# bobzhangbo2012/gnss-sdr-new

Measured on AMD Instinct MI355X. Metric: IQ Msamples/s processed (acq+track), 32 PRN × 81 Doppler; % HBM roofline, higher is better.
Workload: dtype f32; 1 GPU; C2: GPS L1 C/A 4 Msps; per 1 ms block a 32 PRN x 81 Doppler (+-10 kHz, 250 Hz) CFAR PCPS grid + closed-loop DLL/PLL tracking (3-tap E-P-L, dll_pll_veml_tracking) of 8 channels over the same span; fs_sps=4000000, fft_size=4000, prns=32, doppler_bins=81, channels=8, taps=3, item_type=gr_complex, tracking=one continuous stream, one launch per timed region, acq_chains=2, acq_stagger=0, acq_input=each step acquires its own span of the continuous stream (new HBM addresses), carrier=exact, forward_spectra_per_block=4

## Files before the change

gnss-sdr-new_amd/csrc/acq.hip:

```cpp
#include <algorithm>
#include <cmath>
#include <cstring>
#include <memory>
#include <new>
#include <utility>

#include "acq_handle.h"
#include "acq_plans.h"
#include "gsdr_stream_internal.h"

using namespace gsdr_acq_impl;

namespace
{

int dispatch(gsdr_acq* a, const AcqView& v, const AcqOp& op)
{
    if (a->variant >= 20) return dispatch_four(a, v, op);
    if (a->variant >= 10) return dispatch_runtime(a, v, op);
    return dispatch_static(a, v, op);
}

int run_blocks(gsdr_acq* a, const AcqView& v, const void* iq, uint32_t nblocks, uint64_t stride, uint64_t stamp0,
    gsdr_acq_result* res, hipStream_t s)
// ... 4 lines not shown
int run_ring(gsdr_acq* a, gsdr_stream* ring, uint64_t first_sample, uint32_t nblocks, uint64_t stamp0)
{
    gsdr::StreamReader rd(ring);
    const void* iq = nullptr;
    int rc = rd.view(first_sample, (uint64_t)nblocks * a->K * a->consumed, &iq);
    if (rc == GSDR_OK) rc = rd.acquire(a->stream);
    if (rc == GSDR_OK) rc = run_blocks(a, view_of(a), iq, nblocks, a->consumed, stamp0, a->d_res, a->stream);
    if (rc == GSDR_OK) rc = rd.release(a->stream);
    return rc;
}

int read_results(gsdr_acq* a, gsdr_acq_result* out, size_t n)
{
    GSDR_HIP(hipMemcpyAsync(out, a->d_res, n * sizeof(gsdr_acq_result), hipMemcpyDeviceToHost, a->stream));
    GSDR_HIP(hipStreamSynchronize(a->stream));
    return GSDR_OK;
}

int code_fft(gsdr_acq* a, uint32_t first_slot, uint32_t nslots)
{
    AcqOp op{AcqOp::CodeFft};
    op.first_slot = first_slot;
    op.nslots = nslots;
    return dispatch(a, view_of(a), op);
}

void step_two_freqs(const gsdr_acq* a, float center, float* freqs)
{
    const uint32_t nb = a->st2.nbins;
    const float half = (float)std::floor((double)nb / 2.0);
    for (uint32_t d = 0; d < nb; ++d)
        {
            volatile float dop = ((float)d - half) * a->st2.step;
            freqs[d] = center + dop;
        }
}

hipError_t upload_twiddles(float2* d_tw, uint32_t n)
{
    std::vector<float2> tw(n);
    for (uint32_t m = 0; m < n; ++m)
        {
            const double ang = 2.0 * M_PI * (double)m / (double)n;
            tw[m] = make_float2((float)std::cos(ang), (float)(-std::sin(ang)));
        }
    return hipMemcpy(d_tw, tw.data(), (size_t)n * sizeof(float2), hipMemcpyHostToDevice);
}
// ... 102 lines not shown
            a->eff = N / 2;
        }
    a->general = a->K > 1 || conf->bit_transition_flag;
    a->D = conf->num_doppler_bins;
    if (a->D == 0)
        a->D = (uint32_t)std::ceil((double)(conf->doppler_max - (-conf->doppler_max)) / (double)conf->doppler_step);
    GSDR_REQUIRE(a->D != 0, GSDR_E_ARG, "gsdr_acq_create: zero Doppler bins");
    const bool ok = choose_variant(a);
    const bool four = a->variant >= 20;
    a->lds_bytes = (size_t)(four ? a->plan4.sub.n : N) * sizeof(float2) + 16 * sizeof(RowStat);
    GSDR_REQUIRE(ok && a->lds_bytes <= kLdsBytes, GSDR_E_UNSUPPORTED,
        "gsdr_acq_create: FFT size %u not supported (needs 2^a*3^b*5^c; up to 20352 points in LDS, larger sizes as "
        "R*N2 with R in {8,10,12,16,20,25} and N2 <= 20352)", N);
    int rc = dispatch(a, view_of(a), AcqOp{AcqOp::SetAttrs});
    if (rc == GSDR_OK && four) rc = setup_split(a);
    if (rc == GSDR_OK && !a->general && default_pk_variant(N) > 0)
        rc = setup_corr_variant(a, a->env.corr_variant >= 0 ? a->env.corr_variant : default_pk_variant(N));
    if (rc != GSDR_OK) return rc;
    const size_t nP = conf->max_prns, nB = conf->max_blocks;
    hipError_t e = hipStreamCreateWithFlags(&a->stream, hipStreamNonBlocking);
    if (e == hipSuccess) e = hipMalloc(&a->d_tw, (size_t)N * sizeof(float2));
    if (e == hipSuccess) e = hipMalloc(&a->d_wipe, (size_t)a->D * N * sizeof(float2));
    if (e == hipSuccess) e = hipMalloc(&a->d_code_fft, nP * N * sizeof(float2));
    if (e == hipSuccess) e = hipMalloc(&a->d_code_stage, nP * a->consumed * sizeof(float2));
    if (e == hipSuccess) e = hipMalloc(&a->d_prn, nP * sizeof(uint32_t));
    if (e == hipSuccess) e = hipMalloc(&a->d_X, nB * a->K * a->D * N * sizeof(float2));
    if (e == hipSuccess) e = hipMalloc(&a->d_stats, nB * nP * a->K * a->D * sizeof(RowStat));
    if (e == hipSuccess) e = hipMalloc(&a->d_res, nB * nP * sizeof(gsdr_acq_result));
    if (e == hipSuccess) e = hipMalloc(&a->d_iq, nB * a->K * a->consumed * gsdr::item_bytes(conf->item_type));
    if (a->general)
        {
            const int nslots = 256 * 32 / (a->nt / 64);
            a->acc_words = (nslots + 31) / 32;
            if (e == hipSuccess) e = hipMalloc(&a->d_resk, nB * nP * a->K * sizeof(gsdr_acq_result));
            if (e == hipSuccess) e = hipMalloc(&a->d_acc, (size_t)a->acc_words * 32 * a->eff * sizeof(float));
            if (e == hipSuccess) e = hipMalloc(&a->d_acc_slots, (size_t)a->acc_words * sizeof(uint32_t));
            if (e == hipSuccess) e = hipMemset(a->d_acc_slots, 0, (size_t)a->acc_words * sizeof(uint32_t));
        }
    if (e == hipSuccess) e = hipMalloc(&a->d_grid, (size_t)a->D * N * sizeof(float));
    if (e == hipSuccess && a->split > 0 && !(conf->pfa > 0.0f))
        e = hipMalloc(&a->d_rowbuf, nB * nP * N * sizeof(float));
    if (e == hipSuccess && a->split > 0) e = hipMalloc(&a->d_keys, nB * nP * sizeof(unsigned long long));
    if (e == hipSuccess && a->split > 0) e = hipMalloc(&a->d_psum, nB * nP * 4 * sizeof(float));
    if (e == hipSuccess && a->split > 0) e = hipMalloc(&a->d_fscratch, nB * a->K * a->D * N * sizeof(float2));
    if (four)
        {
// ... 16 lines not shown
    rc = rebuild_wipeoffs(a);
    if (rc != GSDR_OK) return rc;
    compute_threshold(a);
    *out = guard.release();
    return GSDR_OK;
}

void gsdr_acq_destroy(gsdr_acq* a)
{
    if (!a) return;
    gsdr::DeviceGuard g(a->device);
    if (a->stream) (void)hipStreamSynchronize(a->stream);
    for (auto& r : a->prof_recs)
        {
            (void)hipEventDestroy(r.a);
            (void)hipEventDestroy(r.b);
        }
    for (hipEvent_t e : a->prof_pool) (void)hipEventDestroy(e);
    for (int i = 0; i < gsdr_acq::kSubs; ++i)
        {
            if (a->sub_done[i]) (void)hipEventDestroy(a->sub_done[i]);
            if (a->h_res[i]) (void)hipHostFree(a->h_res[i]);
        }
    void* bufs[] = {a->st2.d_wipe, a->st2.d_freq, a->d_tw, a->d_wipe, a->d_code_fft, a->d_code_stage, a->d_prn, a->d_X, a->d_stats, a->d_res,
        a->d_iq, a->d_grid, a->d_rowbuf, a->d_keys, a->d_psum, a->d_fscratch, a->d_dgrid, a->d_tw_sub, a->d_scratch, a->d_slots, a->d_resk, a->d_acc, a->d_acc_slots};
    for (void* p : bufs)
        if (p) (void)hipFree(p);
    if (a->stream) (void)hipStreamDestroy(a->stream);
    delete a;
}

int gsdr_acq_get_dims(const gsdr_acq* a, uint32_t* D, uint32_t* N)
{
    GSDR_REQUIRE(a, GSDR_E_ARG, "gsdr_acq_get_dims: null handle");
    if (D) *D = a->D;
    if (N) *N = a->N;
    return GSDR_OK;
}

int gsdr_acq_get_plan(const gsdr_acq* a, int32_t* variant, int32_t* nthreads, int32_t* r1, int32_t* nstages,
    int32_t radix[8])
{
    GSDR_REQUIRE(a, GSDR_E_ARG, "gsdr_acq_get_plan: null handle");
    static_assert(gsdr::fft::kMaxStages == 8, "gsdr_acq_get_plan reports 8 radices");
    const bool four = a->variant >= 20;
    const Plan& p = four ? a->plan4.sub : a->plan;
    if (variant) *variant = a->variant;
// ... 265 lines not shown
    float* grid_host)
{
    GSDR_REQUIRE(a && iq_host && grid_host, GSDR_E_ARG, "gsdr_acq_dump_grid_step_two: null argument");
    GSDR_REQUIRE(prn_slot < a->nprn, GSDR_E_ARG, "gsdr_acq_dump_grid_step_two: prn_slot %u >= nprn %u", prn_slot,
        a->nprn);
    GSDR_REQUIRE(a->st2.nbins > 0, GSDR_E_STATE, "gsdr_acq_dump_grid_step_two: gsdr_acq_set_step_two first");
    GSDR_REQUIRE(a->st2.nbins <= a->D, GSDR_E_UNSUPPORTED,
        "gsdr_acq_dump_grid_step_two: %u narrow bins exceed the grid buffer's %u rows", a->st2.nbins, a->D);
    std::lock_guard<std::mutex> lk(a->mu);
    gsdr::DeviceGuard g(a->device);
    const uint32_t nb = a->st2.nbins;
    std::vector<float> freqs(nb);
    step_two_freqs(a, doppler_center_hz, freqs.data());
    GSDR_HIP(hipMemcpyAsync(a->d_iq, iq_host, (size_t)a->consumed * gsdr::item_bytes(a->conf.item_type),
        hipMemcpyHostToDevice, a->stream));
    GSDR_HIP(hipMemcpyAsync(a->st2.d_freq, freqs.data(), nb * sizeof(float), hipMemcpyHostToDevice, a->stream));
    int rc = launch_wipeoff(a, a->st2.d_wipe, nb, a->st2.d_freq);
    if (rc != GSDR_OK) return rc;
    AcqView v = view_of(a);
    v.D = nb;
    v.nprn = 1;
    v.wipe = a->st2.d_wipe;
    v.code_fft = a->d_code_fft + (size_t)prn_slot * a->N;
    v.xm = XMap{nb, 0u, a->N};
    rc = dispatch(a, v, AcqOp{AcqOp::DumpGrid});
    if (rc != GSDR_OK) return rc;
    GSDR_HIP(hipMemcpyAsync(grid_host, a->d_grid, (size_t)nb * a->N * sizeof(float), hipMemcpyDeviceToHost,
        a->stream));
    GSDR_HIP(hipStreamSynchronize(a->stream));
    return GSDR_OK;
}

int gsdr_acq_set_step_two(gsdr_acq* a, uint32_t num_doppler_bins_step2, float doppler_step2, float pfa2)
{
    GSDR_REQUIRE(a, GSDR_E_ARG, "gsdr_acq_set_step_two: null handle");
    GSDR_REQUIRE(num_doppler_bins_step2 > 0, GSDR_E_ARG, "gsdr_acq_set_step_two: zero bins");
    GSDR_REQUIRE(num_doppler_bins_step2 <= a->D * a->conf.max_blocks, GSDR_E_UNSUPPORTED,
        "gsdr_acq_set_step_two: %u bins exceed the handle's spectrum capacity (%u bins x %u blocks)",
        num_doppler_bins_step2, a->D, a->conf.max_blocks);
    std::lock_guard<std::mutex> lk(a->mu);
    gsdr::DeviceGuard g(a->device);
    GSDR_HIP(hipStreamSynchronize(a->stream));
    if (a->st2.d_wipe) (void)hipFree(a->st2.d_wipe);
    if (a->st2.d_freq) (void)hipFree(a->st2.d_freq);
    a->st2.d_wipe = nullptr;
    a->st2.d_freq = nullptr;
// ... 19 lines not shown
{
    GSDR_REQUIRE(a && iq_host && prn_slots && doppler_center_hz && coarse_input_power && out, GSDR_E_ARG,
        "gsdr_acq_run_step_two: null argument");
    GSDR_REQUIRE(a->st2.nbins > 0, GSDR_E_STATE, "gsdr_acq_run_step_two: gsdr_acq_set_step_two first");
    GSDR_REQUIRE(nsel > 0 && nsel <= a->nprn, GSDR_E_ARG, "gsdr_acq_run_step_two: %u PRNs outside [1,%u]", nsel,
        a->nprn);
    for (uint32_t i = 0; i < nsel; ++i)
        GSDR_REQUIRE(prn_slots[i] < a->nprn, GSDR_E_ARG, "gsdr_acq_run_step_two: slot %u >= nprn %u", prn_slots[i],
            a->nprn);
    std::lock_guard<std::mutex> lk(a->mu);
    gsdr::DeviceGuard g(a->device);
    const uint32_t nb = a->st2.nbins;
    std::vector<float> freqs((size_t)nsel * nb);
    for (uint32_t i = 0; i < nsel; ++i) step_two_freqs(a, doppler_center_hz[i], freqs.data() + (size_t)i * nb);
    GSDR_HIP(hipMemcpyAsync(a->d_iq, iq_host, (size_t)a->K * a->consumed * gsdr::item_bytes(a->conf.item_type),
        hipMemcpyHostToDevice, a->stream));
    GSDR_HIP(hipMemcpyAsync(a->st2.d_freq, freqs.data(), freqs.size() * sizeof(float), hipMemcpyHostToDevice,
        a->stream));
    int rc = launch_wipeoff(a, a->st2.d_wipe, nsel * nb, a->st2.d_freq);
    const float thr = step_two_threshold(a);
    for (uint32_t i = 0; i < nsel && rc == GSDR_OK; ++i)
        {
            const AcqView v{nb, 1, a->st2.d_wipe + (size_t)i * nb * a->N, a->d_code_fft + (size_t)prn_slots[i] * a->N,
                a->d_prn + prn_slots[i], XMap{nb, 0u, a->N}, true, doppler_center_hz[i], coarse_input_power[i], thr};
            rc = run_blocks(a, v, a->d_iq, 1, a->consumed, stamp, a->d_res + i, a->stream);
        }
    if (rc != GSDR_OK) return rc;
    return read_results(a, out, nsel);
}

int gsdr_acq_set_cu_mask(gsdr_acq* a, const uint32_t* mask, int n_words)
{
    GSDR_REQUIRE(a, GSDR_E_ARG, "gsdr_acq_set_cu_mask: null handle");
    std::lock_guard<std::mutex> lk(a->mu);
    gsdr::DeviceGuard g(a->device);
    return gsdr::replace_stream(&a->stream, mask, n_words);
}

int gsdr_acq_set_profiling(gsdr_acq* a, int enable)
{
    GSDR_REQUIRE(a, GSDR_E_ARG, "gsdr_acq_set_profiling: null handle");
    std::lock_guard<std::mutex> lk(a->mu);
    a->profiling = enable != 0;
    if (a->profiling)
        {
            gsdr::DeviceGuard g(a->device);
            while (a->prof_pool.size() + 2 * a->prof_recs.size() < 1024)
// ... 96 lines not shown
```

gnss-sdr-new_amd/csrc/acq_common.hip:

```cpp
#include <cmath>
#include <cstdlib>
#include <string>

#include "acq_handle.h"

namespace
{

__device__ __forceinline__ float2 cephes_sincos_avx2(float x0)
{
    const float FOPI = 1.27323954473516f;
    const float DP1 = -0.78515625f, DP2 = -2.4187564849853515625e-4f, DP3 = -3.77489497744594108e-8f;
    const float C0 = 2.443315711809948E-005f, C1 = -1.388731625493765E-003f, C2 = 4.166664568298827E-002f;
    const float S0 = -1.9515295891E-4f, S1 = 8.3321608736E-3f, S2 = -1.6666654611E-1f;
    const uint32_t bits = __float_as_uint(x0);
    bool sign_sin = (bits >> 31) != 0;
    float x = __uint_as_float(bits & 0x7fffffffu);
    float y = __fmul_rn(x, FOPI);
    int32_t j = (int32_t)y;
    j = (j + 1) & ~1;
    y = (float)j;
    const bool swap = (j & 4) != 0;
    const bool poly = (j & 2) == 0;
    x = __fadd_rn(x, __fmul_rn(y, DP1));
// ... 152 lines not shown
                    const float acc = s[opp].sum;
                    const float ip = ap.step_two ? ap.ip2
                                                 : (float)((double)(acc / (float)(int32_t)ap.eff) / 2.0 / (double)(k + 1));
                    r.input_power = ip;
                    r.test_statistic = m / ip;
                    r.positive = r.test_statistic > ap.threshold ? 1 : 0;
                    done = r.positive || k + 1 == K;
                    if (done && threadIdx.x == 0) res[bp] = r;
                }
            if (threadIdx.x == 0) resk[(size_t)bp * K + k] = r;
        }
}

__global__ void acq_decide_kernel(const gsdr_acq_result* __restrict__ resk, gsdr_acq_result* __restrict__ res,
    uint32_t K, uint32_t n)
{
    const uint32_t bp = blockIdx.x * blockDim.x + threadIdx.x;
    if (bp >= n) return;
    uint32_t k = 0;
    while (k + 1 < K && !resk[(size_t)bp * K + k].positive) ++k;
    res[bp] = resk[(size_t)bp * K + k];
}

__global__ void __launch_bounds__(256) acq_grid_second_peak_kernel(const float* __restrict__ grid,
    gsdr_acq_result* __restrict__ res, AcqParams ap)
{
    __shared__ RowStat scratch[4];
    const uint32_t p = blockIdx.x;
    const uint32_t d = res[p].doppler_index;
    const int32_t ti = (int32_t)res[p].code_phase;
    const int32_t E = (int32_t)ap.N;
    int32_t e1 = ti - (int32_t)ap.samples_per_chip;
    int32_t e2 = ti + (int32_t)ap.samples_per_chip;
    if (e1 < 0)
        e1 = E + e1;
    else if (e2 >= E)
        e2 = e2 - E;
    const float* row = grid + ((size_t)p * ap.D + d) * ap.eff;
    float best = 0.0f, sum = 0.0f;
    uint32_t bidx = 0;
    for (uint32_t j = threadIdx.x; j < ap.eff; j += 256)
        {
            const int32_t jj = (int32_t)j;
            const bool excluded = (e1 < e2) ? (jj >= e1 && jj < e2) : (jj >= e1 || jj < e2);
            const float m = excluded ? 0.0f : row[j];
            if (stat_better(m, j, best, bidx))
// ... 90 lines not shown
#define GSDR_ACQ_QPW_DEFAULT 2
#endif

AcqEnv read_acq_env()
{
    AcqEnv e;
    if (const char* w = std::getenv("GSDR_ACQ_WIPE"))
        {
            const std::string m(w);
            e.wipe_mode = m == "generic" ? GSDR_WIPE_GENERIC : (m == "avx2" ? GSDR_WIPE_AVX2 : GSDR_WIPE_EXACT);
        }
    e.xshift = env_int("GSDR_ACQ_XSHIFT", 1) != 0;
    e.four_generic = env_int("GSDR_ACQ_FOUR_GENERIC", 0) != 0;
    e.split = env_int("GSDR_ACQ_SPLIT", 1) != 0;
    e.split_arg = env_int("GSDR_ACQ_SPLIT_ARG", 1) != 0;
    e.qpw = env_int("GSDR_ACQ_QPW", GSDR_ACQ_QPW_DEFAULT);
    e.ppw = env_int("GSDR_ACQ_PPW", GSDR_ACQ_PPW_DEFAULT);
    e.corr_variant = env_int("GSDR_ACQ_CORR_VARIANT", -1);
    return e;
}

AcqView view_of(const gsdr_acq* a)
{
    return AcqView{a->D, a->nprn, a->d_wipe, a->d_code_fft, a->d_prn, a->xm, false, 0.0f, 0.0f, 0.0f};
}

AcqParams params_of(const gsdr_acq* a, const AcqView& v)
{
    AcqParams ap{};
    ap.xm = v.xm;
    ap.N = a->N;
    ap.consumed = a->consumed;
    ap.lead_zeros = a->lead;
    ap.D = v.D;
    ap.P = v.nprn;
    ap.doppler_max = a->conf.doppler_max;
    ap.doppler_center = a->conf.doppler_center;
    ap.doppler_step = (int32_t)a->conf.doppler_step;
    ap.samples_per_code = a->conf.samples_per_code;
    ap.samples_per_chip = a->conf.samples_per_chip;
    ap.dwells = a->K;
    ap.threshold = a->threshold;
    ap.cfar = a->conf.pfa > 0.0f ? 1 : 0;
    ap.eff = a->eff;
    ap.out_off = a->N - a->eff;
    ap.counter = a->K;
    if (v.step_two)
// ... 51 lines not shown
    return GSDR_OK;
}

int launch_reduce(gsdr_acq* a, const AcqParams& ap, bool dwells, uint32_t nblocks, gsdr_acq_result* res,
    const uint32_t* prn, uint64_t stamp0, uint64_t stride, hipStream_t s)
{
    if (dwells)
        hipLaunchKernelGGL(acq_reduce_dwell_kernel, dim3(nblocks * ap.P), dim3(64), 0, s, a->d_stats, a->d_resk, res,
            prn, ap, stamp0, stride);
    else
        hipLaunchKernelGGL(acq_reduce_kernel, dim3(nblocks * ap.P), dim3(64), 0, s, a->d_stats, res, prn, ap, stamp0,
            stride);
    GSDR_HIP(hipGetLastError());
    return GSDR_OK;
}

int launch_decide(gsdr_acq* a, uint32_t n, gsdr_acq_result* res, hipStream_t s)
{
    hipLaunchKernelGGL(acq_decide_kernel, dim3((n + 255) / 256), dim3(256), 0, s, a->d_resk, res, a->K, n);
    GSDR_HIP(hipGetLastError());
    return GSDR_OK;
}

int launch_grid_second_peak(gsdr_acq* a, const AcqParams& ap, gsdr_acq_result* res, hipStream_t s)
{
    hipLaunchKernelGGL(acq_grid_second_peak_kernel, dim3(ap.P), dim3(256), 0, s, a->d_dgrid, res, ap);
    GSDR_HIP(hipGetLastError());
    return GSDR_OK;
}

void compute_threshold(gsdr_acq* a)
{
    const float pfa = a->conf.pfa;
    if (pfa <= 0.0f) return;
    const int num_bins = (int)(a->eff * a->D);
    const double p = std::pow(1.0 - (double)pfa, 1.0 / (double)(float)num_bins);
    a->threshold = (float)(2.0 * gsdr::gamma_p_inv_int(2 * (int)a->conf.max_dwells, p));
}

float step_two_threshold(const gsdr_acq* a)
{
    const float pfa = a->st2.pfa2;
    if (pfa <= 0.0f) return a->threshold;
    const int num_bins = (int)(a->eff * a->st2.nbins);
    const double p = std::pow(1.0 - (double)pfa, 1.0 / (double)(float)num_bins);
    return (float)(2.0 * gsdr::gamma_p_inv_int(2 * (int)a->conf.max_dwells, p));
// ... 4 lines not shown
```

gnss-sdr-new_amd/csrc/acq_handle.h:

```cpp
#pragma once
#include <mutex>
#include <type_traits>
#include <vector>

#include "acq_kernels.h"

struct AcqEnv
{
    int wipe_mode{GSDR_WIPE_EXACT};
    bool xshift{true}, four_generic{false}, split{true}, split_arg{true};
    int qpw{0}, ppw{0};
    int corr_variant{-1};
};

struct gsdr_acq
{
    int device{0};
    gsdr_acq_conf conf{};
    AcqEnv env{};
    uint32_t N{0}, D{0}, consumed{0}, lead{0};
    uint32_t K{1};
    int wipe_mode{GSDR_WIPE_EXACT};
    gsdr_acq_impl::XMap xm{};
    uint32_t eff{0};
    bool general{false};
    gsdr_acq_result* d_resk{nullptr};
    float* d_acc{nullptr};
    uint32_t* d_acc_slots{nullptr};
    int acc_words{0};
    float threshold{0.0f};
    int nt{256};
    int variant{0};
    int corr_variant{0};
    int split{0};
    int corr_stat{0};
    size_t corr_lds_bytes{0};
    gsdr::fft::Plan plan{};
    gsdr::fft::Plan4 plan4{};
    size_t lds_bytes{0};
    hipStream_t stream{nullptr};
    float2* d_tw{nullptr};
    float2* d_wipe{nullptr};
    float2* d_code_fft{nullptr};
    float2* d_code_stage{nullptr};
    uint32_t* d_prn{nullptr};
    uint32_t nprn{0};
    float2* d_X{nullptr};
    gsdr_acq_impl::RowStat* d_stats{nullptr};
    gsdr_acq_result* d_res{nullptr};
    static constexpr int kSubs = 2;
    gsdr_acq_result* h_res[kSubs]{};
    hipEvent_t sub_done[kSubs]{};
    uint32_t sub_blocks[kSubs]{}, sub_nprn[kSubs]{};
    int sub_head{0}, sub_count{0};
    void* d_iq{nullptr};
    float* d_grid{nullptr};
    float* d_rowbuf{nullptr};
    unsigned long long* d_keys{nullptr};
    float* d_psum{nullptr};
    float2* d_fscratch{nullptr};
    float* d_dgrid{nullptr};
    float2* d_tw_sub{nullptr};
    float2* d_scratch{nullptr};
    uint32_t* d_slots{nullptr};
    struct ProfRec
    {
// ... 2 lines not shown
    };
    bool profiling{false};
    std::vector<ProfRec> prof_recs;
    std::vector<hipEvent_t> prof_pool;
    struct StepTwo
    {
        uint32_t nbins{0};
        float step{0.0f};
        float pfa2{0.0f};
        float2* d_wipe{nullptr};
        float* d_freq{nullptr};
    } st2;
    std::mutex mu;
};

namespace gsdr_acq_impl
{

struct AcqView
{
    uint32_t D, nprn;
    const float2* wipe;
    const float2* code_fft;
    const uint32_t* prn;
    XMap xm;
    bool step_two;
    float center2, ip2, threshold2;
};

struct AcqOp
{
    enum Kind
    {
        Run,
        CodeFft,
        DumpSpectra,
        DumpGrid,
        SetAttrs,
        Dwell
    } kind;
    const void* iq{nullptr};
    uint32_t nblocks{0};
    uint64_t stride{0}, stamp0{0};
    gsdr_acq_result* res{nullptr};
    hipStream_t s{nullptr};
    uint32_t first_slot{0}, nslots{0}, prn_slot{0}, dwell{0};
};

inline int default_pk_variant(uint32_t N)
{
    switch (N)
        {
        case 4000: return 97;
        case 16000: return 94;
        case 8000: return 61;
        case 2000: return 62;
        default: return 0;
        }
}

template <class F>
auto with_item_type(int it, F&& f)
{
    if (it == GSDR_ITEM_GR_COMPLEX) return f(std::integral_constant<int, GSDR_ITEM_GR_COMPLEX>{});
    if (it == GSDR_ITEM_CSHORT) return f(std::integral_constant<int, GSDR_ITEM_CSHORT>{});
    return f(std::integral_constant<int, GSDR_ITEM_IBYTE>{});
}
constexpr int kItemTypes[] = {GSDR_ITEM_GR_COMPLEX, GSDR_ITEM_CSHORT, GSDR_ITEM_IBYTE};

inline int set_max_lds(const void* kernel, size_t bytes)
{
    GSDR_HIP(hipFuncSetAttribute(kernel, hipFuncAttributeMaxDynamicSharedMemorySize, (int)bytes));
    return GSDR_OK;
}

AcqEnv read_acq_env();
AcqView view_of(const gsdr_acq* a);
AcqParams params_of(const gsdr_acq* a, const AcqView& v);
int rebuild_wipeoffs(gsdr_acq* a);
void compute_threshold(gsdr_acq* a);
float step_two_threshold(const gsdr_acq* a);
int launch_wipeoff(gsdr_acq* a, float2* wipe, uint32_t rows, const float* freqs);
int launch_reduce(gsdr_acq* a, const AcqParams& ap, bool dwells, uint32_t nblocks, gsdr_acq_result* res,
    const uint32_t* prn, uint64_t stamp0, uint64_t stride, hipStream_t s);
int launch_decide(gsdr_acq* a, uint32_t n, gsdr_acq_result* res, hipStream_t s);
int launch_grid_second_peak(gsdr_acq* a, const AcqParams& ap, gsdr_acq_result* res, hipStream_t s);

int launch_corr_variant(gsdr_acq* a, const AcqView& v, uint32_t nblocks, hipStream_t s);
int launch_argmax_variant(gsdr_acq* a, const AcqView& v, uint32_t nblocks, gsdr_acq_result* res, hipStream_t s);
int launch_forward_pk(gsdr_acq* a, const AcqView& v, const void* iq, uint32_t nblocks, uint64_t stride, hipStream_t s);
int setup_corr_variant(gsdr_acq* a, int id);
int setup_split(gsdr_acq* a);
int launch_split(gsdr_acq* a, const AcqView& v, uint32_t nblocks, hipStream_t s);
int launch_split_argmax(gsdr_acq* a, const AcqView& v, uint32_t nblocks, gsdr_acq_result* res, hipStream_t s);
int dispatch_static(gsdr_acq* a, const AcqView& v, const AcqOp& op);
int dispatch_runtime(gsdr_acq* a, const AcqView& v, const AcqOp& op);
int dispatch_four(gsdr_acq* a, const AcqView& v, const AcqOp& op);

}
```

gnss-sdr-new_amd/csrc/acq_kernels.h:

```cpp
#pragma once
#include <hip/hip_runtime.h>

#include <type_traits>

#include "fft_4step.h"
#include "fft_lds.h"
#include "fft_multi.h"
#include "fft_pk.h"
#include "fft_plan.h"
#include "gsdr_internal.h"

namespace gsdr_acq_impl
{

struct RowStat
{
    float max;
    uint32_t idx;
    float sum;
    uint32_t pad;
};

struct XMap
{
// ... 268 lines not shown
    };
    auto store = [&](int i, float2 v) {
        const float m = v.x * v.x + v.y * v.y;
        if (GRID) grid[(size_t)d * N + i] = m;
        if (stat_better(m, (uint32_t)i, best, bidx))
            {
                best = m;
                bidx = (uint32_t)i;
            }
        sum += m;
    };
    PT::run(plan, lds, tw, load, store);
    if (!GRID)
        {
            block_reduce_stat<PT::NT>(best, bidx, sum, scratch);
            if (threadIdx.x == 0) stats[((size_t)b * P + p) * D + d] = RowStat{best, bidx, sum, 0};
        }
}

enum CodeSrc
{
    kCodeVgpr = 0,
    kCodeDirect = 1,
    kCodeLds = 2
};

template <class MP, int CS>
constexpr size_t pk_fft_bytes()
{
    constexpr size_t piece = (size_t)(MP::NT / 64) * 1024;
    return CS == kCodeLds ? (MP::lds_bytes() + piece - 1) / piece * piece : MP::lds_bytes();
}

template <class MP, int PG, int WPE, int STAT, int CS>
__global__ void __launch_bounds__(MP::NT) __attribute__((amdgpu_waves_per_eu(WPE))) acq_correlate_pk_kernel(const float2* __restrict__ X,
    const float2* __restrict__ code_fft, RowStat* __restrict__ stats, const float2* __restrict__ tw, uint32_t D,
    uint32_t P, uint32_t nblocks, XMap xm)
{
    static_assert(PG > 0, "PRN group");
    static_assert(CS == kCodeVgpr || CS == kCodeDirect || CS == kCodeLds, "code source");
    constexpr bool PREFETCH = CS == kCodeVgpr;
    constexpr bool STAGED = CS == kCodeLds;
    constexpr int XT = STAGED ? (MP::R1 + 4) / 5 : 0;
    static_assert(STAT == 1 || STAT == 2, "row statistic 1 (max + sum) or 2 (max)");
    using gsdr::pk::c2;
    constexpr int NT = MP::NT;
    constexpr int NW = NT / 64;
    constexpr int R1 = MP::R1, BPT1 = MP::BPT1, NB1 = MP::NB1;
    constexpr uint32_t N = MP::N;
    extern __shared__ float2 lds_raw[];
    c2* lds = reinterpret_cast<c2*>(lds_raw);
    RowStat* scratch = reinterpret_cast<RowStat*>(lds_raw + pk_fft_bytes<MP, CS>() / sizeof(float2));
    const uint32_t G = (P + PG - 1) / PG;
    const uint32_t nrows = nblocks * D;
    const uint32_t id = blockIdx.x;
    const uint32_t full = nrows >> 3;
    uint32_t row, g;
    if (id < full * 8u * G)
        {
            const uint32_t xcd = id & 7u, slot = id >> 3;
            row = (slot / G) * 8u + xcd;
            g = slot - (slot / G) * G;
        }
    else
        {
            const uint32_t t = id - full * 8u * G;
// ... 29 lines not shown
                }
        }
    auto stage_code = [&](int qn) {
        constexpr int PIECE = NW * 1024;
        constexpr int PIECES = (int)(pk_fft_bytes<MP, CS>() / PIECE);
        const int wave = __builtin_amdgcn_readfirstlane((int)(threadIdx.x >> 6));
        char* dst = reinterpret_cast<char*>(lds_raw) + wave * 1024;
        const int voff = (int)threadIdx.x * 16;
#pragma unroll
        for (int k = 0; k < PIECES; ++k)
            __builtin_amdgcn_raw_ptr_buffer_load_lds(crs, (gsdr_lvoid*)(dst + k * PIECE), 16, voff,
                qn * (int)(N * 8) + k * PIECE, 0, 0);
    };
    if constexpr (STAGED)
        {
            stage_code(0);
            asm volatile("s_waitcnt vmcnt(0)" ::: "memory");
            __syncthreads();
        }
    for (int q = 0; q < np; ++q)
        {
            {
                    float rmax = 0.0f, sum = 0.0f;
                    if constexpr (STAGED)
                        {
#pragma unroll
                            for (int bb = 0; bb < BPT1; ++bb)
                                {
                                    const int jj = min((int)threadIdx.x + bb * NT, NB1 - 1);
#pragma unroll
                                    for (int r = R1 - XT; r < R1; ++r) xr[bb][r] = bload(xrs, jj * 8, r * NB1 * 8);
                                }
                            __builtin_amdgcn_sched_barrier(0);
                        }
                    auto load = [&](int bb, int r, int i) -> c2 {
                        if constexpr (PREFETCH)
                            return gsdr::pk::conj_mul(xr[bb][r], cr[bb][r]);
                        else if constexpr (STAGED)
                            {
                                if (XT > 0 && r == R1 - XT) __builtin_amdgcn_sched_barrier(0);
                                return gsdr::pk::conj_mul(xr[bb][r], lds[i]);
                            }
                        else
                            return gsdr::pk::conj_mul(xr[bb][r], bload(crs, i * 8, (int)(q * N * 8)));
                    };
                    auto hook = [&]() {
                        if (PREFETCH && q + 1 < np)
                            {
#pragma unroll
                                for (int bb = 0; bb < BPT1; ++bb)
                                    {
                                        const int j = (int)threadIdx.x + bb * NT;
                                        if (NB1 % NT == 0 || j < NB1)
                                            {
#pragma unroll
                                                for (int r = 0; r < R1; ++r)
                                                    cr[bb][r] = bload(crs, j * 8, (int)((q + 1) * N * 8) + r * NB1 * 8);
                                            }
                                    }
                            }
                    };
                    auto store = [&](int, c2 v, int) {
                        const float m = __builtin_fmaf(v.x, v.x, v.y * v.y);
                        rmax = __builtin_fmaxf(rmax, m);
                        if constexpr (STAT == 1) sum += m;
                    };
                    if constexpr (STAGED)
                        {
                            auto pre = [&]() { __syncthreads(); };
                            auto mid = [&]() {
                                if (q + 1 < np) stage_code(q + 1);
                            };
                            MP::template run<false>(lds, tw, load, store, hook, pre, mid);
                        }
                    else
                        MP::template run<false>(lds, tw, load, store, hook);
                    rmax = gsdr::wave_max(rmax);
                    if constexpr (STAT == 1)
                        {
#pragma unroll
                            for (int off = 32; off > 0; off >>= 1) sum += __shfl_xor(sum, off);
                        }
                    RowStat* sc = scratch + (q & 1) * NW;
                    const int lane = threadIdx.x & 63, wave = threadIdx.x >> 6;
                    if (lane == 0) sc[wave] = RowStat{rmax, 0u, sum, 0};
                    if constexpr (STAGED) asm volatile("s_waitcnt vmcnt(0)" ::: "memory");
                    __syncthreads();
                    if (threadIdx.x == 0)
                        {
                            RowStat best = sc[0];
#pragma unroll
                            for (int w = 1; w < NW; ++w)
                                {
                                    best.max = __builtin_fmaxf(best.max, sc[w].max);
                                    best.sum += sc[w].sum;
                                }
// ... 556 lines not shown
```

gnss-sdr-new_amd/csrc/acq_pk.hip:

```cpp
#include "acq_handle.h"
#include "acq_plans.h"
#include "acq_split_kernels.h"

namespace gsdr_acq_impl
{
namespace
{

using RegPlan93 = RegFourStep<16, 512, 8, 1 | (16 << 4), NoPads<1000>, 10, 10, 10>;
using RegPlan94 = RegFourStep<16, 512, 0, 1 | (16 << 4), NoPads<1000>, 10, 10, 10>;

template <int ID, class MP, int PG_, int WPE_, int ST, class REG = void, int CS_ = kCodeVgpr>
struct PkVariant
{
    static constexpr int id = ID, PG = PG_, WPE = WPE_, STAT = ST, CS = CS_;
    using type = MP;
    using Reg = REG;
};
using PkVariants = PlanList<PkVariant<61, PkPlan<512, true, 20, 20, 20>, 1, 1, 1>,
    PkVariant<62, PkPlan<256, true, 20, 10, 10>, 1, 1, 1>,
    PkVariant<93, PkPlan<1024, 1, 16, 10, 10, 10>, 1, 1, 2, RegPlan93>,
    PkVariant<94, PkPlan<1024, 1, 16, 10, 10, 10>, 1, 1, 2, RegPlan94>,
    PkVariant<70, PkPlan<256, 1, 25, 16, 10>, 1, 1, 2>,
    PkVariant<97, PkPlan<256, 1, 25, 16, 10>, 16, 4, 2, void, kCodeLds>>;

template <class F>
int with_pk_variant(int id, F&& f, int unknown = GSDR_E_STATE)
{
    int rc = unknown;
    const bool found = find_plan(PkVariants{}, [&](auto e) {
        if (decltype(e)::id != id) return false;
        rc = f(e);
        return true;
    });
    if (!found && unknown != GSDR_OK) gsdr::set_error("internal: bad correlate variant %d", id);
    return rc;
}

}

int launch_corr_variant(gsdr_acq* a, const AcqView& v, uint32_t nblocks, hipStream_t s)
{
    return with_pk_variant(a->corr_variant, [&](auto e) {
        using V = decltype(e);
        using M = typename V::type;
        if constexpr (!std::is_void<typename V::Reg>::value)
            {
                using RP = typename V::Reg;
                hipLaunchKernelGGL((acq_correlate_reg_kernel<RP>), dim3(nblocks * v.D * v.nprn), dim3(RP::NT),
                    RP::lds_bytes(), s, a->d_X, v.code_fft, a->d_stats, a->d_tw, v.D, v.nprn, nblocks, v.xm);
            }
        else
            {
                const uint32_t groups = (v.nprn + V::PG - 1) / V::PG;
                hipLaunchKernelGGL((acq_correlate_pk_kernel<M, V::PG, V::WPE, V::STAT, V::CS>), dim3(nblocks * v.D * groups),
                    dim3(M::NT), a->corr_lds_bytes, s, a->d_X, v.code_fft, a->d_stats, a->d_tw, v.D, v.nprn, nblocks,
                    v.xm);
            }
        return GSDR_OK;
    });
}

int launch_argmax_variant(gsdr_acq* a, const AcqView& v, uint32_t nblocks, gsdr_acq_result* res, hipStream_t s)
{
    return with_pk_variant(a->corr_variant, [&](auto e) {
        using V = decltype(e);
        using M = typename V::type;
        hipLaunchKernelGGL((acq_argmax_pk_kernel<M, V::STAT>), dim3(nblocks * v.nprn), dim3(M::NT), a->corr_lds_bytes,
            s, a->d_X, v.code_fft, res, a->d_tw, v.D, v.nprn, a->conf.samples_per_code, params_of(a, v));
        GSDR_HIP(hipGetLastError());
        return GSDR_OK;
    });
}

int launch_forward_pk(gsdr_acq* a, const AcqView& v, const void* iq, uint32_t nblocks, uint64_t stride, hipStream_t s)
{
    return with_pk_variant(a->corr_variant, [&](auto e) {
        using M = typename decltype(e)::type;
        with_item_type(a->conf.item_type, [&](auto t) {
// ... 7 lines not shown

int setup_corr_variant(gsdr_acq* a, int id)
{
    a->corr_variant = 0;
    return with_pk_variant(id, [&](auto e) {
        using V = decltype(e);
        using M = typename V::type;
        if (M::N != (int)a->N)
            {
                gsdr::set_error("correlate variant %d is for N = %d, not %u", V::id, M::N, a->N);
                return GSDR_E_UNSUPPORTED;
            }
        a->corr_lds_bytes = pk_fft_bytes<M, V::CS>() + (size_t)2 * (M::NT / 64) * sizeof(RowStat);
        int rc = set_max_lds((const void*)acq_correlate_pk_kernel<M, V::PG, V::WPE, V::STAT, V::CS>, a->corr_lds_bytes);
        rc |= set_max_lds((const void*)acq_argmax_pk_kernel<M, V::STAT>, a->corr_lds_bytes);
        for (int it : kItemTypes)
            rc |= with_item_type(it, [&](auto t) {
                return set_max_lds((const void*)acq_forward_pk_kernel<M, decltype(t)::value>, M::lds_bytes());
            });
        if constexpr (!std::is_void<typename V::Reg>::value)
            rc |= set_max_lds((const void*)acq_correlate_reg_kernel<typename V::Reg>, V::Reg::lds_bytes());
        if (rc != GSDR_OK) return GSDR_E_DEVICE;
        a->corr_variant = V::id;
        a->corr_stat = V::STAT;
        return GSDR_OK;
    }, GSDR_OK);
}

}
```

gnss-sdr-new_amd/csrc/fft_pk.h:

```cpp
#pragma once

#include <hip/hip_runtime.h>

#include <cmath>
#include <type_traits>

#include "fft_lds.h"
#include "fft_multi.h"

namespace gsdr
{
namespace pk
{

typedef float c2 __attribute__((ext_vector_type(2)));

__device__ __forceinline__ c2 from(float2 v) { return c2{v.x, v.y}; }
__device__ __forceinline__ float2 to(c2 v) { return make_float2(v.x, v.y); }

__device__ __forceinline__ c2 mul(c2 a, c2 b)
{
    c2 r, o;
    asm("v_pk_mul_f32 %0, %1, %2 op_sel_hi:[0,1]" : "=v"(r) : "v"(a), "v"(b));
    asm("v_pk_fma_f32 %0, %1, %2, %3 op_sel:[1,1,0] op_sel_hi:[1,0,1] neg_lo:[1,0,0]"
// ... 198 lines not shown
};
template <>
struct Dft<16> : DftCT<4, 4>
{
};
template <>
struct Dft<20> : DftCT<4, 5>
{
};
template <>
struct Dft<25> : DftCT<5, 5>
{
};
template <>
struct Dft<32> : DftCT<4, 8>
{
};

struct NoHook
{
    __device__ __forceinline__ void operator()() const {}
};

template <int R, int NT, int N, int Ns, bool TWP, bool FIRST, bool LAST, bool ORD, class Load, class Store, class Hook,
    class Pre, class Mid>
__device__ __forceinline__ void stage(c2* lds, const float2* __restrict__ tw, Load& load, Store& store, Hook& hook,
    Pre& pre, Mid& mid)
{
    constexpr int BPT = fft::bpt_for(R);
    constexpr bool PRE = FIRST && !LAST && !std::is_same<Pre, NoHook>::value;
    constexpr bool MID = LAST && !FIRST && TWP && !std::is_same<Mid, NoHook>::value;
    constexpr int NB = N / R;
    constexpr int TSTRIDE = N / (Ns * R);
    c2 v[BPT][R];
    c2 w1[BPT];
    if constexpr (MID)
        {
#pragma unroll
            for (int b = 0; b < BPT; ++b) w1[b] = from(tw[(min(threadIdx.x + (unsigned)(b * NT), (unsigned)(NB - 1)) % Ns) * TSTRIDE]);
        }
#pragma unroll
    for (int b = 0; b < BPT; ++b)
        {
            const int j = (int)threadIdx.x + b * NT;
            if constexpr (BPT == 1 && NB % NT != 0)
                {
                    const int jj = min(j, NB - 1);
#pragma unroll
                    for (int r = 0; r < R; ++r)
                        {
                            if constexpr (FIRST)
                                v[b][r] = load(b, r, jj + r * NB);
                            else
                                v[b][r] = lds[jj + r * NB];
                        }
                }
            else if (NB % NT == 0 || j < NB)
                {
#pragma unroll
                    for (int r = 0; r < R; ++r)
                        {
                            if constexpr (FIRST)
                                v[b][r] = load(b, r, j + r * NB);
                            else
                                v[b][r] = lds[j + r * NB];
                        }
                }
        }
    if constexpr (FIRST)
        hook();
    else
        {
            if constexpr (MID)
                {
#pragma unroll
                    for (int b = 0; b < BPT; ++b) asm volatile("" : "+v"(w1[b]));
                }
// ... 56 lines not shown
                            const int j = (int)threadIdx.x + b * NT;
                            if (NB % NT == 0 || j < NB) store(j + r * Ns, v[b][r], r * BPT + b);
                        }
                }
        }
    else if constexpr (LAST)
        {
            static_assert(!LAST || Ns * R == N, "last stage");
#pragma unroll
            for (int b = 0; b < BPT; ++b)
                {
                    const int j = (int)threadIdx.x + b * NT;
                    if (NB % NT == 0 || j < NB)
                        {
#pragma unroll
                            for (int r = 0; r < R; ++r) store(j + r * Ns, v[b][r], r * BPT + b);
                        }
                }
        }
    else
        __syncthreads();
}

template <int NT, int N, int Ns, bool TWP, bool FIRST, bool ORD, int R, int... Rest, class Load, class Store, class Hook,
    class Pre, class Mid>
__device__ __forceinline__ void stages(c2* lds, const float2* __restrict__ tw, Load& load, Store& store, Hook& hook,
    Pre& pre, Mid& mid)
{
    constexpr bool LAST = sizeof...(Rest) == 0;
    stage<R, NT, N, Ns, TWP, FIRST, LAST, ORD>(lds, tw, load, store, hook, pre, mid);
    if constexpr (!LAST) stages<NT, N, Ns * R, TWP, false, ORD, Rest...>(lds, tw, load, store, hook, pre, mid);
}

template <int NT_, int TWP_, int... Rs>
struct PkPlan
{
    static constexpr int NT = NT_;
    static constexpr bool TWP = TWP_ != 0;
    static constexpr int N = (Rs * ...);
    static constexpr int nstages = sizeof...(Rs);
    static constexpr int R1 = fft::FirstRadix<Rs...>::value;
    static constexpr int BPT1 = fft::bpt_for(R1);
    static constexpr int NB1 = N / R1;
    static constexpr size_t lds_bytes() { return (size_t)N * sizeof(c2); }
    static constexpr int RL = (0, ..., Rs);
    static constexpr int BPTL = fft::bpt_for(RL);
    static constexpr int NSL = N / RL;
    static constexpr int NSLOTS = RL * BPTL;
    __device__ __forceinline__ static int index_of_slot(int slot)
    {
        return (int)threadIdx.x + (slot % BPTL) * NT + (slot / BPTL) * NSL;
    }
    template <bool ORD = true, class Load, class Store, class Hook, class Pre = NoHook, class Mid = NoHook>
    __device__ __forceinline__ static void run(c2* lds, const float2* __restrict__ tw, Load load, Store store, Hook hook,
        Pre pre = Pre{}, Mid mid = Mid{})
    {
        stages<NT, N, 1, TWP, true, ORD, Rs...>(lds, tw, load, store, hook, pre, mid);
    }
};


}
}
```

Before: 250.0 Msamples/s.

## Add lane-ordered code spectrum variant for N=4000 correlation first stage

Adds a second copy of each PRN's code FFT, permuted so that each thread's R1 first-stage inputs sit contiguously in LDS. The new correlation variant 98 reads them as double-buffered groups of five instead of strided LDS loads, and it drops the extra code-staging pre-hook. It also skips first-stage loads for whole wavefronts beyond NB1. It is now the default for N=4000. The cost is an extra permutation kernel after each code FFT and an extra device buffer, and the design relies on a constexpr bijectivity check.

```diff
diff --git a/gnss-sdr-new_amd/csrc/acq.hip b/gnss-sdr-new_amd/csrc/acq.hip
--- a/gnss-sdr-new_amd/csrc/acq.hip
+++ b/gnss-sdr-new_amd/csrc/acq.hip
@@ -50,7 +50,9 @@
     AcqOp op{AcqOp::CodeFft};
     op.first_slot = first_slot;
     op.nslots = nslots;
-    return dispatch(a, view_of(a), op);
+    const int rc = dispatch(a, view_of(a), op);
+    if (rc != GSDR_OK || !a->d_code_lane) return rc;
+    return launch_code_lane_order(a, first_slot, nslots);
 }
 
 void step_two_freqs(const gsdr_acq* a, float center, float* freqs)
@@ -199,6 +201,7 @@
     if (e == hipSuccess) e = hipMalloc(&a->d_tw, (size_t)N * sizeof(float2));
     if (e == hipSuccess) e = hipMalloc(&a->d_wipe, (size_t)a->D * N * sizeof(float2));
     if (e == hipSuccess) e = hipMalloc(&a->d_code_fft, nP * N * sizeof(float2));
+    if (e == hipSuccess && a->lane_nb1 > 0) e = hipMalloc(&a->d_code_lane, nP * N * sizeof(float2));
     if (e == hipSuccess) e = hipMalloc(&a->d_code_stage, nP * a->consumed * sizeof(float2));
     if (e == hipSuccess) e = hipMalloc(&a->d_prn, nP * sizeof(uint32_t));
     if (e == hipSuccess) e = hipMalloc(&a->d_X, nB * a->K * a->D * N * sizeof(float2));
@@ -261,7 +264,7 @@
             if (a->sub_done[i]) (void)hipEventDestroy(a->sub_done[i]);
             if (a->h_res[i]) (void)hipHostFree(a->h_res[i]);
         }
-    void* bufs[] = {a->st2.d_wipe, a->st2.d_freq, a->d_tw, a->d_wipe, a->d_code_fft, a->d_code_stage, a->d_prn, a->d_X, a->d_stats, a->d_res,
+    void* bufs[] = {a->st2.d_wipe, a->st2.d_freq, a->d_tw, a->d_wipe, a->d_code_fft, a->d_code_lane, a->d_code_stage, a->d_prn, a->d_X, a->d_stats, a->d_res,
         a->d_iq, a->d_grid, a->d_rowbuf, a->d_keys, a->d_psum, a->d_fscratch, a->d_dgrid, a->d_tw_sub, a->d_scratch, a->d_slots, a->d_resk, a->d_acc, a->d_acc_slots};
     for (void* p : bufs)
         if (p) (void)hipFree(p);
@@ -573,6 +576,7 @@
     v.nprn = 1;
     v.wipe = a->st2.d_wipe;
     v.code_fft = a->d_code_fft + (size_t)prn_slot * a->N;
+    v.code_lane = a->d_code_lane ? a->d_code_lane + (size_t)prn_slot * a->N : nullptr;
     v.xm = XMap{nb, 0u, a->N};
     rc = dispatch(a, v, AcqOp{AcqOp::DumpGrid});
     if (rc != GSDR_OK) return rc;
@@ -638,7 +642,7 @@
     for (uint32_t i = 0; i < nsel && rc == GSDR_OK; ++i)
         {
             const AcqView v{nb, 1, a->st2.d_wipe + (size_t)i * nb * a->N, a->d_code_fft + (size_t)prn_slots[i] * a->N,
-                a->d_prn + prn_slots[i], XMap{nb, 0u, a->N}, true, doppler_center_hz[i], coarse_input_power[i], thr};
+                a->d_code_lane ? a->d_code_lane + (size_t)prn_slots[i] * a->N : nullptr, a->d_prn + prn_slots[i], XMap{nb, 0u, a->N}, true, doppler_center_hz[i], coarse_input_power[i], thr};
             rc = run_blocks(a, v, a->d_iq, 1, a->consumed, stamp, a->d_res + i, a->stream);
         }
     if (rc != GSDR_OK) return rc;
diff --git a/gnss-sdr-new_amd/csrc/acq_common.hip b/gnss-sdr-new_amd/csrc/acq_common.hip
--- a/gnss-sdr-new_amd/csrc/acq_common.hip
+++ b/gnss-sdr-new_amd/csrc/acq_common.hip
@@ -198,6 +198,14 @@
     res[bp] = resk[(size_t)bp * K + k];
 }
 
+__global__ void __launch_bounds__(256) acq_code_lane_order_kernel(const float2* __restrict__ src,
+    float2* __restrict__ dst, uint32_t N, int nb1, int r1)
+{
+    const float2* in = src + (size_t)blockIdx.x * N;
+    float2* out = dst + (size_t)blockIdx.x * N;
+    for (uint32_t i = threadIdx.x; i < N; i += blockDim.x) out[lane_order_slot((int)i, nb1, r1)] = in[i];
+}
+
 __global__ void __launch_bounds__(256) acq_grid_second_peak_kernel(const float* __restrict__ grid,
     gsdr_acq_result* __restrict__ res, AcqParams ap)
 {
@@ -334,7 +342,7 @@
 
 AcqView view_of(const gsdr_acq* a)
 {
-    return AcqView{a->D, a->nprn, a->d_wipe, a->d_code_fft, a->d_prn, a->xm, false, 0.0f, 0.0f, 0.0f};
+    return AcqView{a->D, a->nprn, a->d_wipe, a->d_code_fft, a->d_code_lane, a->d_prn, a->xm, false, 0.0f, 0.0f, 0.0f};
 }
 
 AcqParams params_of(const gsdr_acq* a, const AcqView& v)
@@ -432,6 +440,15 @@
     return GSDR_OK;
 }
 
+int launch_code_lane_order(gsdr_acq* a, uint32_t first_slot, uint32_t nslots)
+{
+    const size_t off = (size_t)first_slot * a->N;
+    hipLaunchKernelGGL(acq_code_lane_order_kernel, dim3(nslots), dim3(256), 0, a->stream, a->d_code_fft + off,
+        a->d_code_lane + off, a->N, a->lane_nb1, a->lane_r1);
+    GSDR_HIP(hipGetLastError());
+    return GSDR_OK;
+}
+
 int launch_grid_second_peak(gsdr_acq* a, const AcqParams& ap, gsdr_acq_result* res, hipStream_t s)
 {
     hipLaunchKernelGGL(acq_grid_second_peak_kernel, dim3(ap.P), dim3(256), 0, s, a->d_dgrid, res, ap);
diff --git a/gnss-sdr-new_amd/csrc/acq_handle.h b/gnss-sdr-new_amd/csrc/acq_handle.h
--- a/gnss-sdr-new_amd/csrc/acq_handle.h
+++ b/gnss-sdr-new_amd/csrc/acq_handle.h
@@ -35,6 +35,7 @@
     int split{0};
     int corr_stat{0};
     size_t corr_lds_bytes{0};
+    int lane_nb1{0}, lane_r1{0};
     gsdr::fft::Plan plan{};
     gsdr::fft::Plan4 plan4{};
     size_t lds_bytes{0};
@@ -42,6 +43,7 @@
     float2* d_tw{nullptr};
     float2* d_wipe{nullptr};
     float2* d_code_fft{nullptr};
+    float2* d_code_lane{nullptr};
     float2* d_code_stage{nullptr};
     uint32_t* d_prn{nullptr};
     uint32_t nprn{0};
@@ -90,6 +92,7 @@
     uint32_t D, nprn;
     const float2* wipe;
     const float2* code_fft;
+    const float2* code_lane;
     const uint32_t* prn;
     XMap xm;
     bool step_two;
@@ -119,7 +122,7 @@
 {
     switch (N)
         {
-        case 4000: return 97;
+        case 4000: return 98;
         case 16000: return 94;
         case 8000: return 61;
         case 2000: return 62;
@@ -153,6 +156,7 @@
     const uint32_t* prn, uint64_t stamp0, uint64_t stride, hipStream_t s);
 int launch_decide(gsdr_acq* a, uint32_t n, gsdr_acq_result* res, hipStream_t s);
 int launch_grid_second_peak(gsdr_acq* a, const AcqParams& ap, gsdr_acq_result* res, hipStream_t s);
+int launch_code_lane_order(gsdr_acq* a, uint32_t first_slot, uint32_t nslots);
 
 int launch_corr_variant(gsdr_acq* a, const AcqView& v, uint32_t nblocks, hipStream_t s);
 int launch_argmax_variant(gsdr_acq* a, const AcqView& v, uint32_t nblocks, gsdr_acq_result* res, hipStream_t s);
diff --git a/gnss-sdr-new_amd/csrc/acq_kernels.h b/gnss-sdr-new_amd/csrc/acq_kernels.h
--- a/gnss-sdr-new_amd/csrc/acq_kernels.h
+++ b/gnss-sdr-new_amd/csrc/acq_kernels.h
@@ -314,14 +314,26 @@
 {
     kCodeVgpr = 0,
     kCodeDirect = 1,
-    kCodeLds = 2
+    kCodeLds = 2,
+    kCodeLane = 3
 };
+
+constexpr int lane_order_slot(int i, int nb1, int r1) { return (i % nb1) * r1 + i / nb1; }
+constexpr bool lane_order_bijective(int nb1, int r1)
+{
+    for (int i = 0; i < nb1 * r1; ++i)
+        {
+            const int s = lane_order_slot(i, nb1, r1);
+            if (s < 0 || s >= nb1 * r1 || (s % r1) * nb1 + s / r1 != i) return false;
+        }
+    return true;
+}
 
 template <class MP, int CS>
 constexpr size_t pk_fft_bytes()
 {
     constexpr size_t piece = (size_t)(MP::NT / 64) * 1024;
-    return CS == kCodeLds ? (MP::lds_bytes() + piece - 1) / piece * piece : MP::lds_bytes();
+    return CS == kCodeLds || CS == kCodeLane ? (MP::lds_bytes() + piece - 1) / piece * piece : MP::lds_bytes();
 }
 
 template <class MP, int PG, int WPE, int STAT, int CS>
@@ -330,10 +342,13 @@
     uint32_t P, uint32_t nblocks, XMap xm)
 {
     static_assert(PG > 0, "PRN group");
-    static_assert(CS == kCodeVgpr || CS == kCodeDirect || CS == kCodeLds, "code source");
+    static_assert(CS == kCodeVgpr || CS == kCodeDirect || CS == kCodeLds || CS == kCodeLane, "code source");
     constexpr bool PREFETCH = CS == kCodeVgpr;
-    constexpr bool STAGED = CS == kCodeLds;
-    constexpr int XT = STAGED ? (MP::R1 + 4) / 5 : 0;
+    constexpr bool LANE = CS == kCodeLane;
+    constexpr bool STAGED = CS == kCodeLds || LANE;
+    static_assert(!LANE || (MP::BPT1 == 1 && lane_order_bijective(MP::NB1, MP::R1)), "lane order of the first stage");
+    constexpr int XT = CS == kCodeLds ? (MP::R1 + 4) / 5 : 0;
+    constexpr int RA = LANE ? 5 : 0;
     static_assert(STAT == 1 || STAT == 2, "row statistic 1 (max + sum) or 2 (max)");
     using gsdr::pk::c2;
     constexpr int NT = MP::NT;
@@ -409,7 +424,7 @@
         {
             {
                     float rmax = 0.0f, sum = 0.0f;
-                    if constexpr (STAGED)
+                    if constexpr (XT > 0)
                         {
 #pragma unroll
                             for (int bb = 0; bb < BPT1; ++bb)
@@ -420,12 +435,31 @@
                                 }
                             __builtin_amdgcn_sched_barrier(0);
                         }
+                    c2 cb[2][RA > 0 ? RA : 1];
                     auto load = [&](int bb, int r, int i) -> c2 {
                         if constexpr (PREFETCH)
                             return gsdr::pk::conj_mul(xr[bb][r], cr[bb][r]);
                         else if constexpr (STAGED)
                             {
                                 if (XT > 0 && r == R1 - XT) __builtin_amdgcn_sched_barrier(0);
+                                if constexpr (LANE)
+                                    {
+                                        const c2* row = lds + min((int)threadIdx.x, NB1 - 1) * R1;
+                                        if (r % RA == 0)
+                                            {
+                                                if (r == 0)
+                                                    {
+#pragma unroll
+                                                        for (int k = 0; k < RA; ++k) cb[0][k] = row[k];
+                                                    }
+                                                const int g = r / RA + 1;
+#pragma unroll
+                                                for (int k = 0; k < RA; ++k)
+                                                    if (g * RA + k < R1) cb[g & 1][k] = row[g * RA + k];
+                                                __builtin_amdgcn_sched_barrier(0);
+                                            }
+                                        return gsdr::pk::conj_mul(xr[bb][r], cb[(r / RA) & 1][r % RA]);
+                                    }
                                 return gsdr::pk::conj_mul(xr[bb][r], lds[i]);
                             }
                         else
@@ -458,7 +492,10 @@
                             auto mid = [&]() {
                                 if (q + 1 < np) stage_code(q + 1);
                             };
-                            MP::template run<false>(lds, tw, load, store, hook, pre, mid);
+                            if constexpr (LANE)
+                                MP::template run<false, true>(lds, tw, load, store, hook, gsdr::pk::NoHook{}, mid);
+                            else
+                                MP::template run<false>(lds, tw, load, store, hook, pre, mid);
                         }
                     else
                         MP::template run<false>(lds, tw, load, store, hook);
diff --git a/gnss-sdr-new_amd/csrc/acq_pk.hip b/gnss-sdr-new_amd/csrc/acq_pk.hip
--- a/gnss-sdr-new_amd/csrc/acq_pk.hip
+++ b/gnss-sdr-new_amd/csrc/acq_pk.hip
@@ -22,7 +22,8 @@
     PkVariant<93, PkPlan<1024, 1, 16, 10, 10, 10>, 1, 1, 2, RegPlan93>,
     PkVariant<94, PkPlan<1024, 1, 16, 10, 10, 10>, 1, 1, 2, RegPlan94>,
     PkVariant<70, PkPlan<256, 1, 25, 16, 10>, 1, 1, 2>,
-    PkVariant<97, PkPlan<256, 1, 25, 16, 10>, 16, 4, 2, void, kCodeLds>>;
+    PkVariant<97, PkPlan<256, 1, 25, 16, 10>, 16, 4, 2, void, kCodeLds>,
+    PkVariant<98, PkPlan<256, 1, 25, 16, 10>, 16, 4, 2, void, kCodeLane>>;
 
 template <class F>
 int with_pk_variant(int id, F&& f, int unknown = GSDR_E_STATE)
@@ -54,7 +55,7 @@
             {
                 const uint32_t groups = (v.nprn + V::PG - 1) / V::PG;
                 hipLaunchKernelGGL((acq_correlate_pk_kernel<M, V::PG, V::WPE, V::STAT, V::CS>), dim3(nblocks * v.D * groups),
-                    dim3(M::NT), a->corr_lds_bytes, s, a->d_X, v.code_fft, a->d_stats, a->d_tw, v.D, v.nprn, nblocks,
+                    dim3(M::NT), a->corr_lds_bytes, s, a->d_X, V::CS == kCodeLane ? v.code_lane : v.code_fft, a->d_stats, a->d_tw, v.D, v.nprn, nblocks,
                     v.xm);
             }
         return GSDR_OK;
@@ -108,6 +109,8 @@
             rc |= set_max_lds((const void*)acq_correlate_reg_kernel<typename V::Reg>, V::Reg::lds_bytes());
         if (rc != GSDR_OK) return GSDR_E_DEVICE;
         a->corr_variant = V::id;
+        a->lane_nb1 = V::CS == kCodeLane ? M::NB1 : 0;
+        a->lane_r1 = V::CS == kCodeLane ? M::R1 : 0;
         a->corr_stat = V::STAT;
         return GSDR_OK;
     }, GSDR_OK);
diff --git a/gnss-sdr-new_amd/csrc/fft_pk.h b/gnss-sdr-new_amd/csrc/fft_pk.h
--- a/gnss-sdr-new_amd/csrc/fft_pk.h
+++ b/gnss-sdr-new_amd/csrc/fft_pk.h
@@ -244,8 +244,8 @@
     __device__ __forceinline__ void operator()() const {}
 };
 
-template <int R, int NT, int N, int Ns, bool TWP, bool FIRST, bool LAST, bool ORD, class Load, class Store, class Hook,
-    class Pre, class Mid>
+template <int R, int NT, int N, int Ns, bool TWP, bool FIRST, bool LAST, bool ORD, bool SKIPW, class Load, class Store,
+    class Hook, class Pre, class Mid>
 __device__ __forceinline__ void stage(c2* lds, const float2* __restrict__ tw, Load& load, Store& store, Hook& hook,
     Pre& pre, Mid& mid)
 {
@@ -268,13 +268,16 @@
             if constexpr (BPT == 1 && NB % NT != 0)
                 {
                     const int jj = min(j, NB - 1);
-#pragma unroll
-                    for (int r = 0; r < R; ++r)
-                        {
-                            if constexpr (FIRST)
-                                v[b][r] = load(b, r, jj + r * NB);
-                            else
-                                v[b][r] = lds[jj + r * NB];
+                    if (!FIRST || !SKIPW || __builtin_amdgcn_readfirstlane((int)(threadIdx.x & ~63u)) < NB)
+                        {
+#pragma unroll
+                            for (int r = 0; r < R; ++r)
+                                {
+                                    if constexpr (FIRST)
+                                        v[b][r] = load(b, r, jj + r * NB);
+                                    else
+                                        v[b][r] = lds[jj + r * NB];
+                                }
                         }
                 }
             else if (NB % NT == 0 || j < NB)
@@ -377,14 +380,14 @@
         __syncthreads();
 }
 
-template <int NT, int N, int Ns, bool TWP, bool FIRST, bool ORD, int R, int... Rest, class Load, class Store, class Hook,
-    class Pre, class Mid>
+template <int NT, int N, int Ns, bool TWP, bool FIRST, bool ORD, bool SKIPW, int R, int... Rest, class Load, class Store,
+    class Hook, class Pre, class Mid>
 __device__ __forceinline__ void stages(c2* lds, const float2* __restrict__ tw, Load& load, Store& store, Hook& hook,
     Pre& pre, Mid& mid)
 {
     constexpr bool LAST = sizeof...(Rest) == 0;
-    stage<R, NT, N, Ns, TWP, FIRST, LAST, ORD>(lds, tw, load, store, hook, pre, mid);
-    if constexpr (!LAST) stages<NT, N, Ns * R, TWP, false, ORD, Rest...>(lds, tw, load, store, hook, pre, mid);
+    stage<R, NT, N, Ns, TWP, FIRST, LAST, ORD, SKIPW>(lds, tw, load, store, hook, pre, mid);
+    if constexpr (!LAST) stages<NT, N, Ns * R, TWP, false, ORD, SKIPW, Rest...>(lds, tw, load, store, hook, pre, mid);
 }
 
 template <int NT_, int TWP_, int... Rs>
@@ -406,14 +409,14 @@
     {
         return (int)threadIdx.x + (slot % BPTL) * NT + (slot / BPTL) * NSL;
     }
-    template <bool ORD = true, class Load, class Store, class Hook, class Pre = NoHook, class Mid = NoHook>
+    template <bool ORD = true, bool SKIPW = false, class Load, class Store, class Hook, class Pre = NoHook, class Mid = NoHook>
     __device__ __forceinline__ static void run(c2* lds, const float2* __restrict__ tw, Load load, Store store, Hook hook,
         Pre pre = Pre{}, Mid mid = Mid{})
     {
-        stages<NT, N, 1, TWP, true, ORD, Rs...>(lds, tw, load, store, hook, pre, mid);
-    }
-};
-
-
-}
-}
+        stages<NT, N, 1, TWP, true, ORD, SKIPW, Rs...>(lds, tw, load, store, hook, pre, mid);
+    }
+};
+
+
+}
+}
```

Measured after the change: 265.0 Msamples/s (median of 6 runs). 6.0% higher.
